# DIVE128/DMVSNet

Measured on AMD Instinct MI355X. Metric: depth-maps/sec, DTU 1600x1184 5-view 3-stage (64/32/8 hyp), higher is better.
Workload: dtype f32; 1 GPU; BASELINE configs[1]: 1600x1184, 5 views, 64/32/8 hypotheses, 3 stage(s) x (main + 4-plane refine); parallelism=1 GPU, k1=warp_corr_q4 (quad-planar features, one launch configuration per shape), conv_backend=auto, streams=2, maps_in_flight=1, hip_graph=False

## Files before the change

### dmvsnet_amd/csrc/common.h

```cpp
#pragma once
#include <hip/hip_runtime.h>
#include <stdint.h>
#include "../../include/dmvs.h"

#define DMVS_LAUNCH_CHECK()                         \
    do {                                            \
        hipError_t e__ = hipGetLastError();         \
        return e__ == hipSuccess ? 0 : (int)e__;    \
    } while (0)

static inline int ceil_div(int a, int b) { return (a + b - 1) / b; }

int dmvs_ensure_dynamic_lds(const void* kernel, size_t lds_bytes);

typedef float float4_t __attribute__((ext_vector_type(4)));
typedef float float2_t __attribute__((ext_vector_type(2)));

static inline unsigned xcd_grid(int ntiles) { return 8u * (unsigned)((ntiles + 7) / 8); }

static inline double wino_filter(const double g[9], int i, int p) {
    static const double Gm[4][3] = {{1, 0, 0}, {0.5, 0.5, 0.5}, {0.5, -0.5, 0.5}, {0, 0, 1}};
    double u = 0.0;
    for (int ky = 0; ky < 3; ++ky)
        for (int kx = 0; kx < 3; ++kx) u += Gm[i][ky] * Gm[p][kx] * g[ky * 3 + kx];
    return u;
}

enum { DMVS_ZFORM_S1 = 0, DMVS_ZFORM_S2 = 1, DMVS_ZFORM_T2 = 2 };
#ifdef __HIPCC__
__host__ __device__
#endif
constexpr unsigned zpad_live_mask(int form, int D, int oz0, int TZ) {
    unsigned m = 0;
    for (int p = 0; p < TZ; ++p) {
        const int z = oz0 + p;
        const int nplanes = form == DMVS_ZFORM_S2 ? (D + 1) / 2 : D;
        if (z < 0 || z >= nplanes) continue;
        for (int kz = 0; kz < 3; ++kz) {
            const int iz = form == DMVS_ZFORM_S1 ? z + kz - 1 : form == DMVS_ZFORM_S2 ? 2 * z + kz - 1 : (kz == 0 ? z + 1 : z);
            if (iz >= 0 && iz < D) m |= 1u << (3 * p + kz);
        }
    }
    return m;
}

constexpr int kZpadMaxDepth = 4;
extern long g_zpad_skip;
static inline bool zpad_skip_wanted(int D) { return g_zpad_skip && D <= kZpadMaxDepth; }

#ifdef __HIPCC__
__device__ __forceinline__ bool xcd_tile(int nx, int ny, int nz, bool z_fast, int& bx, int& by, int& bz) {
    const int n = nx * ny * nz, per = (n + 7) >> 3;
    const int id = blockIdx.x, t = (id & 7) * per + (id >> 3);
    if (t >= n) return false;
    bx = t % nx;
    const int r = t / nx;
    if (z_fast) { bz = r % nz; by = r / nz; } else { by = r % ny; bz = r / ny; }
    return true;
}
#endif
```

### dmvsnet_amd/csrc/conv3d_mfma.hip

```cpp
#ifndef DMVS_KO
#define DMVS_KO 0
#endif
#ifndef DMVS_X
#define DMVS_X 0
#endif
#include "common.h"
#include "tile_loader.h"

#include <algorithm>
#include <cstdlib>
#include <mutex>


#include <map>
#include <type_traits>
#include <utility>

int dmvs_ensure_dynamic_lds(const void* kernel, size_t lds_bytes) {
    static std::mutex mu;
    static std::map<std::pair<int, const void*>, size_t> configured;
    int dev = 0;
    if (hipGetDevice(&dev) != hipSuccess) return (int)hipGetLastError();
    std::lock_guard<std::mutex> lock(mu);
    auto key = std::make_pair(dev, kernel);
// ... 61 lines not shown
    }
    static __device__ __forceinline__ int row(int r, int lk) { return lk * 4 + r; }
};

template <int NROWS>
__device__ __forceinline__ void load_weights(__amdgpu_buffer_rsrc_t rs_w, float* wl, int chunk, int wave, int lane) {
    constexpr int NI = (NROWS + 3) / 4;
    const unsigned base = (unsigned)chunk * NROWS * 256u + (unsigned)lane * 16u;
#pragma unroll
    for (int r = 0; r < (NI + 3) / 4; ++r) {
        const int j = min(wave + 4 * r, NI - 1);
        if (j * 256 + lane * 4 < NROWS * 64)
            __builtin_amdgcn_raw_ptr_buffer_load_lds(rs_w, (lds_ptr_t)(wl + j * 256), 16, base + (unsigned)j * 1024u, 0, 0, 0);
    }
}

template <int M, int STRIDE, int KD, int KS, int CI_CH, int TZ, int TY, bool V4>
struct ConvGeom {
    static constexpr int KK = Frag<M>::KK;
    static constexpr int NT = KS * KS * KD;
    static constexpr int IZ = KD == 3 ? (TZ - 1) * STRIDE + 3 : TZ, IY = (TY - 1) * STRIDE + KS, IX = 31 * STRIDE + KS;
    static constexpr int XOFF = V4 && KS > 1 ? 4 - KS / 2 : 0;
    static constexpr int IXP = V4 ? (XOFF + IX + 3) / 4 * 4 : IX + 1;
    static constexpr int LPR = IXP / 4;
    static constexpr int PS0 = IZ * IY * IXP;
    static constexpr int BANK = M == 16 ? 16 : 32;
    static constexpr int PS = V4 ? PS0 + (BANK - PS0 % 64 + 64) % 64 : PS0;
    static constexpr int GPC = CI_CH / KK;
    static constexpr int TPG = CI_CH < KK ? KK / CI_CH : 1;
    static constexpr int NSTEPS = CI_CH < KK ? (NT + TPG - 1) / TPG : NT * GPC;
    static constexpr int TILE_F = (CI_CH * PS + 63) & ~63;
};

template <int M, int MB, int STRIDE, int KD, int KS, int CI_CH, int TZ, int TY, int ROWS, bool V4, bool MBS = false, unsigned ZDEAD = 0>
__global__ __launch_bounds__(256, (M == 16 ? 3 : 1)) void conv_mfma_kernel(ConvArgs a) {
    static_assert(!ZDEAD || (KD == 3 && KS == 3), "only the 3x3x3 layers have depth taps");
    typedef Frag<M> F;
    typedef typename F::acc_t acc_t;
    typedef ConvGeom<M, STRIDE, KD, KS, CI_CH, TZ, TY, V4> G;
    constexpr int PAD = KS / 2;
    constexpr int XB = 32 / F::NV;
    constexpr int SZ = KD == 3 ? STRIDE : 1;
    constexpr int IZ = G::IZ, IY = G::IY, IX = G::IX, IXP = G::IXP, PS = G::PS, GPC = G::GPC;
    constexpr int WROWS = G::NSTEPS * MB;
    constexpr int BUF_F = G::TILE_F + WROWS * 64;
    constexpr bool PACKED = CI_CH < F::KK;
    constexpr bool TR = M == 16;
    static_assert(TZ * TY == (MBS ? 2 : 4) * ROWS, "tile rows must equal the row-owning waves x ROWS");
    static_assert(!MBS || MB == 2, "M-block split: two-block layers only");
    constexpr int MBL = MBS ? 1 : MB;
    static_assert(PACKED ? (F::KK % CI_CH == 0) : (CI_CH % F::KK == 0), "channel chunk vs MFMA k-group");
    extern __shared__ __attribute__((aligned(16))) float smem[];

    const int tid = threadIdx.x, lane = tid & 63;
    const int wave = __builtin_amdgcn_readfirstlane(tid >> 6);
    const int ln = lane % F::NV, lk = lane / F::NV;
    const int rwave = MBS ? (wave >> 1) : wave;
    const int mb0 = MBS ? (wave & 1) : 0;
    int bx, by, bz;
    if (!xcd_tile(a.nx, a.ny, a.nz, KD == 3, bx, by, bz)) return;
    const int ox0 = bx * 32, oy0 = by * TY, oz0 = bz * TZ;
    const int ix0 = ox0 * STRIDE - PAD, iy0 = oy0 * STRIDE - PAD, iz0 = KD == 3 ? oz0 * STRIDE - 1 : oz0;
    if (DMVS_X & 8) {
        switch ((blockIdx.x >> 3) & 3) {
            case 1: __builtin_amdgcn_s_setprio(1); break;
            case 2: __builtin_amdgcn_s_setprio(2); break;
            case 3: __builtin_amdgcn_s_setprio(3); break;
            default: break;
        }
// ... 17 lines not shown
        for (int st = 0; st < G::NSTEPS; ++st) {
            int toff = 0;
#pragma unroll
            for (int q = 0; q < TPG; ++q) {
                const int t = st * TPG + q < NT ? st * TPG + q : NT - 1;
                const int o = ((t / (KS * KS)) * IY + (t / KS) % KS) * IXP + t % KS;
                toff = (tsel == q) ? o : toff;
            }
            ptap[st] = boff[0][0] + toff;
            asm volatile("" : "+v"(ptap[st]));
        }
    }

    acc_t acc[MBL][ROWS][XB];
#pragma unroll
    for (int mb = 0; mb < MBL; ++mb)
#pragma unroll
        for (int i = 0; i < ROWS; ++i)
#pragma unroll
            for (int xb = 0; xb < XB; ++xb)
#pragma unroll
                for (int r = 0; r < F::ACC; ++r) acc[mb][i][xb][r] = 0.f;

    const int in_vol = a.D * a.H * a.W;
    auto chunk_rsrc = [&](int ci0, int nch) {
        if (a.in_cs)
            return __builtin_amdgcn_make_buffer_rsrc((void*)(a.in + (size_t)ci0 * a.in_cs), (short)0, (a.in_elems - ci0 * a.in_cs) * 4, 0x00020000);
        return __builtin_amdgcn_make_buffer_rsrc((void*)(a.in + (size_t)ci0 * in_vol), (short)0, nch * in_vol * 4, 0x00020000);
    };
    const int nchunks = a.Cin / CI_CH;
    const __amdgpu_buffer_rsrc_t rs_w =
        __builtin_amdgcn_make_buffer_rsrc((void*)a.w, (short)0, nchunks * WROWS * 256, 0x00020000);

    auto stage = [&](int c, float* dst) {
        if (!(DMVS_KO & 1)) {
            if constexpr (V4)
                load_tile4<CI_CH, IZ, IY, G::LPR, PS>(a.D, a.H, a.W, chunk_rsrc(c * CI_CH, CI_CH), dst, iz0, iy0, ix0 - G::XOFF, wave, lane, a.in_cs, a.in_zs);
            else
                load_tile<CI_CH, IZ, IY, IX, IXP, PS, true>(a.D, a.H, a.W, chunk_rsrc(c * CI_CH, CI_CH), dst, c * CI_CH, iz0, iy0, ix0, wave, lane, a.in_cs, a.in_zs);
        }
        load_weights<WROWS>(rs_w, dst + G::TILE_F, c, wave, lane);
    };
    float sc_tr[TR ? MBL : 1], sh_tr[TR ? MBL : 1];
    if constexpr (TR && !(DMVS_X & 1)) {
#pragma unroll
        for (int mb = 0; mb < MBL; ++mb) {
            const int co = (mb0 + mb) * M + ln;
            const bool cok = co < a.Cout;
            sc_tr[mb] = (a.scale && cok) ? a.scale[co] : 1.f;
            sh_tr[mb] = (a.scale && cok) ? a.shift[co] : 0.f;
        }
    }
    K3_TR(0, K3_NOW());
    K3_TR_HW();
    [[maybe_unused]] unsigned long long tr_wait = 0, tr_mfma = 0, tr_t = K3_NOW();
    stage(0, smem);
    for (int c = 0; c < nchunks; ++c) {
        asm volatile("s_waitcnt vmcnt(0)" ::: "memory");
        __syncthreads();
#ifdef DMVS_K3_TRACE
        { const unsigned long long n = K3_NOW(); tr_wait += n - tr_t; tr_t = n; if (c == 0) K3_TR(1, n); }
#endif
        float* cur = smem + (a.single_buf ? 0 : (c & 1)) * BUF_F;
        if (c + 1 < nchunks && !a.single_buf) {
            stage(c + 1, smem + ((c + 1) & 1) * BUF_F);
        }
        const float* tile = cur;
        const float* wl = cur + G::TILE_F + lane;
        if constexpr (PACKED) {
// ... 451 lines not shown
    {16, 16, DMVS_CONV_S1, 1, 16, 1, CI_F1},
    {16, 32, DMVS_CONV2D_K5S2, 1, 32, 1, CI_K5B},
    {32, 32, DMVS_CONV_S1, 1, 32, 1, CI_F2},
    {32, 16, DMVS_CONV_S1, 1, 16, 1, CI_FO3},
    {32, 64, DMVS_CONV2D_K1, 1, 32, 2, CI_K1},
    {16, 32, DMVS_CONV2D_K1, 1, 32, 1, CI_K1},
    {8, 32, DMVS_CONV2D_K1, 1, 32, 1, CI_K1},
};

int taps_of(int mode, int kdepth) {
    return mode == DMVS_CONV2D_K5S2 ? 25 : mode == DMVS_CONV2D_K1 ? 1 : 9 * kdepth;
}

const Cfg* find_cfg(int cin, int cout, int mode, int kdepth) {
    for (const Cfg& c : kCfgs)
        if (c.cin == cin && c.cout == cout && c.mode == mode && c.kd == kdepth) return &c;
    return nullptr;
}

int tap_of(int p, int o) { return p == 0 ? 1 : (o == 0 ? 2 : 0); }

#define kMinBlocks g_min_blocks

template <typename K>
int launch_with_lds(K kernel, dim3 tiles, size_t lds_bytes, ConvArgs a, hipStream_t st) {
    a.nx = tiles.x; a.ny = tiles.y; a.nz = tiles.z;
    a.st4 = a.Wo % 4 == 0 && (reinterpret_cast<uintptr_t>(a.out) & 15) == 0;
    const dim3 grid(xcd_grid(tiles.x * tiles.y * tiles.z));
    if (int e = dmvs_ensure_dynamic_lds(reinterpret_cast<const void*>(kernel), lds_bytes)) return e;
    kernel<<<grid, 256, lds_bytes, st>>>(a);
    DMVS_LAUNCH_CHECK();
}

template <int M, int MB, int STRIDE, int KD, int KS, int CI_CH, int TZ, int TY, bool V4, bool MBS = false, unsigned ZDEAD = 0>
int launch_conv_tile_v(const ConvArgs& a, hipStream_t st) {
    if constexpr (KD == 3 && KS == 3 && STRIDE == 2 && TZ == 1 && V4 && ZDEAD == 0)
        if (zpad_skip_wanted(a.D) && a.Do == 1 && (~zpad_live_mask(DMVS_ZFORM_S2, a.D, 0, 1) & 7u) == 1u)
            return launch_conv_tile_v<M, MB, STRIDE, KD, KS, CI_CH, TZ, TY, V4, MBS, 1u>(a, st);
    typedef ConvGeom<M, STRIDE, KD, KS, CI_CH, TZ, TY, V4> G;
    constexpr int ROWS = TZ * TY / (MBS ? 2 : 4);
    constexpr size_t lds2 = 2 * (size_t)(G::TILE_F + G::NSTEPS * MB * 64) * sizeof(float);
    static_assert(lds2 <= 160 * 1024, "two pipeline stages must fit the 160 KB LDS");
    ConvArgs b = a;
    dim3 grid(ceil_div(a.Wo, 32), ceil_div(a.Ho, TY), ceil_div(a.Do, TZ));
    b.single_buf = (KD == 3 && (long)grid.x * grid.y * grid.z >= g_single_buf_min_blocks) ? 1 : 0;
    return launch_with_lds(conv_mfma_kernel<M, MB, STRIDE, KD, KS, CI_CH, TZ, TY, ROWS, V4, MBS, ZDEAD>, grid, b.single_buf ? lds2 / 2 : lds2, b, st);
}

inline bool can_v4(const ConvArgs& a) { return a.W % 4 == 0 && (reinterpret_cast<uintptr_t>(a.in) & 15) == 0; }

template <int M, int MB, int STRIDE, int KD, int KS, int CI_CH, int TZ, int TY, bool MBS = false>
int launch_conv_tile(const ConvArgs& a, hipStream_t st) {
    return can_v4(a) ? launch_conv_tile_v<M, MB, STRIDE, KD, KS, CI_CH, TZ, TY, true, MBS>(a, st)
                     : launch_conv_tile_v<M, MB, STRIDE, KD, KS, CI_CH, TZ, TY, false, MBS>(a, st);
}

#define kSplitBlocks g_split_blocks
constexpr int kPlanMBS = 1 << 17;
inline int conv_tile_choice(int stride, int kd, int Do, int Ho, int Wo, int MB) {
    const bool flat = (kd == 1) || Do == 1;
    const int big_ty_flat = (stride == 1) ? 16 : 8, big_ty = (stride == 1) ? 8 : 4;
    const long big_blocks = flat ? (long)ceil_div(Wo, 32) * ceil_div(Ho, big_ty_flat) * Do
                                 : (long)ceil_div(Wo, 32) * ceil_div(Ho, big_ty) * ceil_div(Do, 2);
    const bool big = big_blocks >= kMinBlocks;
    if (!big && MB == 2) {
        const long small_blocks = flat ? (long)ceil_div(Wo, 32) * ceil_div(Ho, 4) * Do
                                       : (long)ceil_div(Wo, 32) * ceil_div(Ho, 2) * ceil_div(Do, 2);
        if (small_blocks < kSplitBlocks) return kPlanMBS | (flat ? 256 + 2 : 2 * 256 + 1);
    }
    if (flat) return 256 + (big ? big_ty_flat : 4);
    return 2 * 256 + (big ? big_ty : 2);
}

template <int M, int MB, int STRIDE, int KD, int CI_CH, int KS = 3>
int launch_conv(const ConvArgs& a, hipStream_t st) {
    constexpr int BIG_TY_FLAT = (STRIDE == 1) ? 16 : 8, BIG_TY = (STRIDE == 1) ? 8 : 4;
    const int choice = conv_tile_choice(STRIDE, KD, a.Do, a.Ho, a.Wo, MB);
    const int tz = (choice >> 8) & 255, ty = choice & 255;
    if constexpr (MB == 2) {
// ... 184 lines not shown
```

### dmvsnet_amd/csrc/conv3d_wino.hip

```cpp
#ifndef DMVS_WKO
#define DMVS_WKO 0
#endif
#include "common.h"
#include "tile_loader.h"
#include "wino.h"
#include "dev_guard.h"

#include <algorithm>
#include <cmath>
#include <vector>

extern long g_wino_stages, g_wino_persistent, g_wino_conv0_grid;
namespace {

constexpr bool kNoStores = (DMVS_WKO & 4) != 0;
#if DMVS_WKO & 2
__device__ __forceinline__ acc4_t wino_mfma(float a, float b, acc4_t c) { c.x += a + b; return c; }
#else
__device__ __forceinline__ acc4_t wino_mfma(float a, float b, acc4_t c) { return __builtin_amdgcn_mfma_f32_16x16x4f32(a, b, c, 0, 0, 0); }
#endif

struct WinoArgs {
    const float* in;
    float* out;
// ... 227 lines not shown
#pragma unroll
                for (int oz = 0; oz < TZ; ++oz)
#pragma unroll
                    for (int t = 0; t < TRW; ++t) {
                        float row[2][8];
#pragma unroll
                        for (int r = 0; r < 4; ++r) wino_out_xform(acc[oz][t][mb], r, row[0] + 2 * r, row[1] + 2 * r);
                        const int oz_g = oz0 + oz;
#pragma unroll
                        for (int rr = 0; rr < 2; ++rr) {
                            const int oy = oy0 + 2 * (TRW * trg + t) + rr;
                            const bool rok = cok && oz_g < a.D && oy < a.H;
#pragma unroll
                            for (int h = 0; h < 2; ++h) {
                                const int x = ox0 + 8 * lk + 4 * h;
                                const unsigned pos = (unsigned)(co * out_vol + oz_g * out_plane + oy * a.W + x) * 4u;
                                v4u_t qv;
                                qv.x = wino_bn_relu(row[rr][4 * h + 0], sc[mb][0], sh[mb][0], lo);
                                qv.y = wino_bn_relu(row[rr][4 * h + 1], sc[mb][0], sh[mb][0], lo);
                                qv.z = wino_bn_relu(row[rr][4 * h + 2], sc[mb][0], sh[mb][0], lo);
                                qv.w = wino_bn_relu(row[rr][4 * h + 3], sc[mb][0], sh[mb][0], lo);
                                wino_store16<kNoStores>(rs_out, qv, (rok && x < a.W) ? pos : kInvalid);
                            }
                        }
                    }
            }
        }
        if (!has_next) break;
        cur = nxt;
        vb += (int)gridDim.x;
    }
}

__global__ __launch_bounds__(256, 2) void conv0_wino_kernel(WinoArgs a) {
    constexpr int TZ = 2, TY = 8, IZ = 4, IY = 10, LPR = 10, IXP = 40;
    constexpr int PS0 = IZ * IY * IXP, PS = PS0 + (32 - PS0 % 64 + 64) % 64;
    constexpr int TILE_F = (2 * PS + 63) & ~63, W_F = 2 * 4 * 256;
    constexpr unsigned kInvalid = kWinoInvalid;
    extern __shared__ __attribute__((aligned(16))) float smem[];

    const int tid = threadIdx.x, lane = tid & 63;
    const int wave = __builtin_amdgcn_readfirstlane(tid >> 6);
    const int ln = lane & 15, lk = lane >> 4;
    struct Tile { int ox0, oy0, oz0; };
    const XcdTileWalk walk(a.nx * a.ny * a.nz);
    auto tile_of = [&](int vb, Tile& t) {
        int id;
        if (!walk.id_of(vb, id)) return false;
        const int bx = id % a.nx, r = id / a.nx;
        t.ox0 = bx * 32; t.oz0 = (r % a.nz) * TZ; t.oy0 = (r / a.nz) * TY;
        return true;
    };
    int vb = blockIdx.x;
    Tile cur, nxt;
    if (!tile_of(vb, cur)) return;

    const int in_vol = a.D * a.H * a.W;
    const __amdgpu_buffer_rsrc_t rs_in = __builtin_amdgcn_make_buffer_rsrc((void*)a.in, (short)0, 2 * in_vol * 4, 0x00020000);
    const __amdgpu_buffer_rsrc_t rs_w = __builtin_amdgcn_make_buffer_rsrc((void*)a.w, (short)0, W_F * 4, 0x00020000);
    float* const tiles = smem + W_F;
    auto stage = [&](const Tile& t, float* dst) {
        if (DMVS_WKO & 1) return;
        load_tile4<2, IZ, IY, LPR, PS>(a.D, a.H, a.W, rs_in, dst, t.oz0 - 1, t.oy0 - 1, t.ox0 - 4, wave, lane);
    };
    const int pbase = (lk & 1) * PS + (2 * wave) * IXP + 2 + 2 * ln;
    const int zsel = lk >> 1;
    const float* wl = smem + lane * 4;

    const int co = ln;
    const float sc = a.scale ? a.scale[co] : 1.f, sh = a.scale ? a.shift[co] : 0.f;
    const int out_plane = a.H * a.W, out_vol = a.D * out_plane;
    const __amdgpu_buffer_rsrc_t rs_out = __builtin_amdgcn_make_buffer_rsrc((void*)a.out, (short)0, a.Cout * out_vol * 4, 0x00020000);
    const float lo = a.relu ? 0.f : -INFINITY;

    load_rows64<W_F / 64>(rs_w, smem, 0, wave, lane);
    stage(cur, tiles);
    for (int k = 0;; ++k) {
        const bool has_next = tile_of(vb + (int)gridDim.x, nxt);
        asm volatile("s_waitcnt vmcnt(0)" ::: "memory");
        __syncthreads();
        if (has_next) stage(nxt, tiles + ((k + 1) & 1) * TILE_F);
        const float* tile = tiles + (k & 1) * TILE_F + pbase;
        acc4_t acc[TZ][16];
#pragma unroll
        for (int oz = 0; oz < TZ; ++oz)
#pragma unroll
            for (int st = 0; st < 2; ++st) {
                const float* p = tile + (oz + (st ? 2 : zsel)) * (IY * IXP);
                float d[4][4];
                wino_read_patch(p, IXP, d);
                float v[16];
#pragma unroll
                for (int x = 0; x < 4; ++x) wino_bt4(d[0][x], d[1][x], d[2][x], d[3][x], d[0][x], d[1][x], d[2][x], d[3][x]);
#pragma unroll
                for (int y = 0; y < 4; ++y) wino_bt4(d[y][0], d[y][1], d[y][2], d[y][3], v[4 * y], v[4 * y + 1], v[4 * y + 2], v[4 * y + 3]);
#pragma unroll
// ... 6 lines not shown
                        acc[oz][4 * q + e] = wino_mfma(v[4 * q + e], wv4[e], c0);
                    }
                }
            }
#pragma unroll
        for (int oz = 0; oz < TZ; ++oz) {
            float row[2][8];
#pragma unroll
            for (int r = 0; r < 4; ++r) wino_out_xform(acc[oz], r, row[0] + 2 * r, row[1] + 2 * r);
            const int oz_g = cur.oz0 + oz;
#pragma unroll
            for (int rr = 0; rr < 2; ++rr) {
                const int oy = cur.oy0 + 2 * wave + rr;
                const bool rok = oz_g < a.D && oy < a.H;
#pragma unroll
                for (int h = 0; h < 2; ++h) {
                    const int x = cur.ox0 + 8 * lk + 4 * h;
                    const unsigned pos = (unsigned)(co * out_vol + oz_g * out_plane + oy * a.W + x) * 4u;
                    v4u_t qv;
                    qv.x = wino_bn_relu(row[rr][4 * h + 0], sc, sh, lo);
                    qv.y = wino_bn_relu(row[rr][4 * h + 1], sc, sh, lo);
                    qv.z = wino_bn_relu(row[rr][4 * h + 2], sc, sh, lo);
                    qv.w = wino_bn_relu(row[rr][4 * h + 3], sc, sh, lo);
                    wino_store16<kNoStores>(rs_out, qv, (rok && x < a.W) ? pos : kInvalid);
                }
            }
        }
        if (!has_next) break;
        cur = nxt;
        vb += (int)gridDim.x;
    }
}

template <bool Q4>
__global__ __launch_bounds__(512, 2) void fpn_wino_kernel(WinoArgs a, const float* ones) {
    constexpr int IY = 18, IXP = 40, LPR = 10, PS = 736, PPP = PS / 4;
    constexpr int TD_IXP = 24, TD_LPR = 6, TD_PS = 240, TD_PPP = 60;
    constexpr int LAT_F = 9 * PS, TD_F = 32 * TD_PS, STAGE_F = LAT_F + TD_F;
    constexpr int WL_F = 3 * 4 * 256, WT_F = 8 * 3 * 256, W_F = WL_F + WT_F;
    constexpr int NI_LAT = (9 * PPP + 63) / 64, NI_TD = (32 * TD_PPP + 63) / 64, NI = NI_LAT + NI_TD;
    static_assert((8 * PPP) % 64 == 0, "the ones plane starts on an instruction boundary");
    constexpr unsigned kInvalid = kWinoInvalid;
    extern __shared__ __attribute__((aligned(16))) float smem[];

    const int tid = threadIdx.x, lane = tid & 63;
    const int wave = __builtin_amdgcn_readfirstlane(tid >> 6);
    const int ln = lane & 15, lk = lane >> 4;
    struct Tile { int ox0, oy0, z; };
    const XcdTileWalk walk(a.nx * a.ny * a.nz);
    auto tile_of = [&](int vb, Tile& t) {
        int id;
        if (!walk.id_of(vb, id)) return false;
        const int bx = id % a.nx, r = id / a.nx;
        t.ox0 = bx * 32; t.oy0 = (r % a.ny) * 16; t.z = r / a.ny;
        return true;
    };
    int vb = blockIdx.x;
    Tile cur, nxt;
    if (!tile_of(vb, cur)) return;

    const int plane = a.H * a.W, in_vol = a.D * plane;
    const int tdH = a.H >> 1, tdW = a.W >> 1, td_plane = tdH * tdW, td_vol = a.D * td_plane;
    const __amdgpu_buffer_rsrc_t rs_lat = __builtin_amdgcn_make_buffer_rsrc((void*)a.lat, (short)0, 8 * in_vol * 4, 0x00020000);
    const __amdgpu_buffer_rsrc_t rs_one = __builtin_amdgcn_make_buffer_rsrc((void*)ones, (short)0, plane * 4, 0x00020000);
    const __amdgpu_buffer_rsrc_t rs_td = __builtin_amdgcn_make_buffer_rsrc((void*)a.td, (short)0, 32 * td_vol * 4, 0x00020000);
    const __amdgpu_buffer_rsrc_t rs_w = __builtin_amdgcn_make_buffer_rsrc((void*)a.w, (short)0, W_F * 4, 0x00020000);
    float* const stages = smem + W_F;
    constexpr int NJ = (NI + 7) / 8;
    int s_rel[NJ], s_rc[NJ];
#pragma unroll
    for (int j = 0; j < NJ; ++j) {
        const int i = wave + 8 * j;
        if (i < NI_LAT) {
            const int p = i * 64 + lane, pl = p / PPP, r = p - pl * PPP, row = r / LPR, pc = r - row * LPR;
            const bool one = i >= 8 * PPP / 64;
            s_rel[j] = (one ? 0 : pl * in_vol) + row * a.W + 4 * pc;
            s_rc[j] = row | (4 * pc) << 8 | ((pl < 9 && row < IY) ? 1 << 16 : 0) | (p < 9 * PPP ? 1 << 17 : 0);
        } else {
            const int it = i - NI_LAT;
            const int p = it * 64 + lane, pl = p / TD_PPP, r = p - pl * TD_PPP, row = r / TD_LPR, pc = r - row * TD_LPR;
            s_rel[j] = pl * td_vol + row * tdW + 4 * pc;
            s_rc[j] = row | (4 * pc) << 8 | ((i < NI && pl < 32) ? 3 << 16 : 0);
        }
    }
    auto stage = [&](const Tile& t, float* dst) {
        if (DMVS_WKO & 1) return;
        const int lat0 = t.z * plane + (t.oy0 - 1) * a.W + t.ox0 - 4, td0 = t.z * td_plane + ((t.oy0 >> 1) - 1) * tdW + (t.ox0 >> 1) - 4;
#pragma unroll
        for (int j = 0; j < NJ; ++j) {
            const int i = wave + 8 * j;
            if (i >= NI) break;
            const int row = s_rc[j] & 255, col = (s_rc[j] >> 8) & 255;
            if (i < NI_LAT) {
                const int gy = t.oy0 - 1 + row, gx = t.ox0 - 4 + col;
                const bool ok = (s_rc[j] & (1 << 16)) && (unsigned)gy < (unsigned)a.H && (unsigned)gx < (unsigned)a.W;
                const bool one = i >= 8 * PPP / 64;
                const unsigned off = ok ? (unsigned)(s_rel[j] + (one ? lat0 - t.z * plane : lat0)) * 4u : kInvalid;
                if (s_rc[j] & (1 << 17)) {
                    if (one) __builtin_amdgcn_raw_ptr_buffer_load_lds(rs_one, (lds_ptr_t)(dst + i * 256), 16, off, 0, 0, 0);
                    else __builtin_amdgcn_raw_ptr_buffer_load_lds(rs_lat, (lds_ptr_t)(dst + i * 256), 16, off, 0, 0, 0);
                }
            } else {
                const int gy = (t.oy0 >> 1) - 1 + row, gx = (t.ox0 >> 1) - 4 + col;
                const bool ok = (s_rc[j] & (1 << 16)) && (unsigned)gy < (unsigned)tdH && (unsigned)gx < (unsigned)tdW;
                __builtin_amdgcn_raw_ptr_buffer_load_lds(rs_td, (lds_ptr_t)(dst + LAT_F + (i - NI_LAT) * 256), 16,
                                                         ok ? (unsigned)(s_rel[j] + td0) * 4u : kInvalid, 0, 0, 0);
            }
        }
    };
    for (int j = wave; j < W_F / 256; j += 8)
        __builtin_amdgcn_raw_ptr_buffer_load_lds(rs_w, (lds_ptr_t)(smem + j * 256), 16, (unsigned)(j * 1024 + lane * 16), 0, 0, 0);

    constexpr int NCO = Q4 ? 4 : 1;
    float sc[NCO], sh[NCO];
#pragma unroll
    for (int r = 0; r < NCO; ++r) {
        const int co = Q4 ? 4 * lk + r : ln;
        sc[r] = a.scale ? a.scale[co] : 1.f;
        sh[r] = a.scale ? a.shift[co] : 0.f;
    }
// ... 124 lines not shown
        vb += (int)gridDim.x;
    }
}

}
long g_wino_stages = 0;
long g_wino_persistent = 1;
long g_wino_conv0_grid = 512;
namespace {

template <int KD, int MB, int MBW, int TZ, int TRW, int GPC, bool Q4 = false, bool ZSKIP = false>
int launch_wino(WinoArgs a, bool single_buf, hipStream_t st) {
    if constexpr (KD == 3 && TZ == 2 && !ZSKIP)
        if (zpad_skip_wanted(a.D)) return launch_wino<KD, MB, MBW, TZ, TRW, GPC, Q4, true>(a, single_buf, st);
    typedef WinoGeom<KD, MB, MBW, TZ, TRW, GPC> G;
    constexpr size_t lds2 = 2 * (size_t)G::BUF_F * sizeof(float);
    static_assert(lds2 / 2 <= 160 * 1024, "one stage must fit the LDS");
    a.nx = ceil_div(a.W, 32); a.ny = ceil_div(a.H, G::TY); a.nz = ceil_div(a.D, TZ);
    if (g_wino_stages) single_buf = g_wino_stages == 1;
    a.single_buf = (single_buf || lds2 > 160 * 1024) ? 1 : 0;
    const size_t lds = a.single_buf ? lds2 / 2 : lds2;
    auto kernel = conv_wino_kernel<KD, MB, MBW, TZ, TRW, GPC, Q4, ZSKIP>;
    if (int e = dmvs_ensure_dynamic_lds(reinterpret_cast<const void*>(kernel), lds)) return e;
    const unsigned resident = 256u * (unsigned)std::max<size_t>(1, std::min<size_t>(2, (160 * 1024) / lds));
    const unsigned grid = std::min(xcd_grid(a.nx * a.ny * a.nz), g_wino_persistent ? resident : 0xffffffffu);
    kernel<<<dim3(grid), 256, lds, st>>>(a);
    DMVS_LAUNCH_CHECK();
}

int launch_conv0_wino(WinoArgs a, bool, hipStream_t st) {
    constexpr int PS0 = 4 * 10 * 40, PS = PS0 + (32 - PS0 % 64 + 64) % 64;
    constexpr size_t lds = (2 * 4 * 256 + 2 * (size_t)((2 * PS + 63) & ~63)) * sizeof(float);
    a.nx = ceil_div(a.W, 32); a.ny = ceil_div(a.H, 8); a.nz = ceil_div(a.D, 2);
    if (int e = dmvs_ensure_dynamic_lds(reinterpret_cast<const void*>(conv0_wino_kernel), lds)) return e;
    const unsigned grid = std::min(xcd_grid(a.nx * a.ny * a.nz), g_wino_persistent ? (unsigned)g_wino_conv0_grid : 0xffffffffu);
    conv0_wino_kernel<<<dim3(grid), 256, lds, st>>>(a);
    DMVS_LAUNCH_CHECK();
}

typedef int (*WinoLaunch)(WinoArgs, bool single_buf, hipStream_t);
struct WCfg {
    int cin, cout, kd;
    bool flat;
    int MB, GPC;
    int TZ, TY;
    bool single_buf;
    WinoLaunch launch[2];
    long ksteps() const { return GPC ? (long)cin / 4 * kd : 2; }
};
template <int KD, int MB, int MBW, int TZ, int TRW, int GPC>
constexpr WCfg wino_row(int cin, int cout, bool flat, bool single_buf) {
    return {cin, cout, KD, flat, MB, GPC, TZ, WinoGeom<KD, MB, MBW, TZ, TRW, GPC>::TY, single_buf,
            {launch_wino<KD, MB, MBW, TZ, TRW, GPC, false>, launch_wino<KD, MB, MBW, TZ, TRW, GPC, true>}};
}
const WCfg kWCfgs[] = {
    wino_row<3, 1, 1, 1, 2, 1>(16, 16, true, true),
    wino_row<3, 1, 1, 2, 1, 1>(16, 16, false, true),
    wino_row<3, 2, 2, 1, 1, 1>(32, 32, false, true),
    wino_row<3, 4, 2, 1, 1, 1>(64, 64, false, true),
    wino_row<1, 4, 2, 1, 1, 1>(64, 64, false, true),
    wino_row<1, 1, 1, 1, 2, 2>(16, 16, false, false),
    wino_row<1, 2, 2, 1, 1, 2>(32, 32, false, false),
    {2, 16, 3, false, 1, 0, 2, 8, false, {launch_conv0_wino, nullptr}},
    wino_row<1, 1, 1, 1, 2, 1>(32, 16, false, false),
};

const WCfg* find_wcfg(int cin, int cout, int kd, int D = 0) {
    for (const WCfg& c : kWCfgs)
        if (c.cin == cin && c.cout == cout && c.kd == kd && (!c.flat || D == 1)) return &c;
// ... 91 lines not shown
    for (int gk = 0; gk < 8; ++gk)
        for (int q = 0; q < 3; ++q)
            for (int l = 0; l < 64; ++l)
                for (int e = 0; e < 4; ++e) {
                    const int j = 4 * q + e, co = l % 16, ci = 4 * gk + l / 16;
                    if (j >= 9) { out[n++] = 0.f; continue; }
                    const int ya = pos[j / 3], xb = pos[j % 3];
                    double g[9];
                    for (int t = 0; t < 9; ++t) g[t] = w3[((size_t)co * Cin + ci) * 9 + t];
                    out[n++] = (float)(wino_filter(g, ya, xb) * (ya == 1 ? 2.0 : 1.0) * (xb == 1 ? 2.0 : 1.0));
                }
    (void)Cout;
    return n == (size_t)dmvs_conv3d_wino_fpn_weight_floats() ? 0 : DMVS_EINVAL;
}

extern "C" int dmvs_conv3d_wino_fpn2(const float* lat, const float* td, const float* ones_hw, float* out, const float* w_packed,
                                     const float* scale, const float* shift, int D, int H, int W, int flags,
                                     dmvs_stream_t stream) {
    if (!lat || !td || !ones_hw || !out || !w_packed || D < 1 || H < 2 || W < 8) return DMVS_EINVAL;
    if ((scale == nullptr) != (shift == nullptr)) return DMVS_EINVAL;
    if (flags & ~(DMVS_RELU | DMVS_OUT_Q4)) return DMVS_EUNSUPPORTED;
    if ((H & 1) || (W & 7)) return DMVS_EUNSUPPORTED;
    if (((reinterpret_cast<uintptr_t>(lat) | reinterpret_cast<uintptr_t>(td) | reinterpret_cast<uintptr_t>(out) |
          reinterpret_cast<uintptr_t>(ones_hw)) & 15) != 0) return DMVS_EUNSUPPORTED;
    if ((long)16 * D * H * W >= (1L << 29)) return DMVS_EUNSUPPORTED;
    WinoArgs a = {};
    a.lat = lat; a.td = td; a.out = out; a.w = w_packed; a.scale = scale; a.shift = shift;
    a.Cin = 32; a.Cout = 16; a.D = D; a.H = H; a.W = W; a.relu = (flags & DMVS_RELU) ? 1 : 0;
    a.nx = ceil_div(W, 32); a.ny = ceil_div(H, 16); a.nz = D;
    constexpr size_t lds = ((3 * 4 + 8 * 3) * 256 + 2 * (size_t)(9 * 736 + 32 * 240)) * sizeof(float);
    static_assert(lds <= 160 * 1024, "filters + two stages must fit the LDS");
    hipStream_t st = (hipStream_t)stream;
    const unsigned grid = std::min(xcd_grid(a.nx * a.ny * a.nz), 256u);
    if (flags & DMVS_OUT_Q4) {
        if (int e = dmvs_ensure_dynamic_lds(reinterpret_cast<const void*>(fpn_wino_kernel<true>), lds)) return e;
        fpn_wino_kernel<true><<<dim3(grid), 512, lds, st>>>(a, ones_hw);
    } else {
        if (int e = dmvs_ensure_dynamic_lds(reinterpret_cast<const void*>(fpn_wino_kernel<false>), lds)) return e;
        fpn_wino_kernel<false><<<dim3(grid), 512, lds, st>>>(a, ones_hw);
    }
    DMVS_LAUNCH_CHECK();
}
```

### dmvsnet_amd/csrc/layout.hip

```cpp
#include "common.h"

#include <cstring>

template <int C>
__global__ __launch_bounds__(256) void nchw_to_hwc_kernel(const float* __restrict__ src, long chan_stride, int c0, int HW,
                                                          float* __restrict__ dst) {
    __shared__ float tile[C * 257];
    const int p0 = blockIdx.x * 256;
    const int t = threadIdx.x;
    const int np = min(256, HW - p0);
    if (t < np) {
#pragma unroll
        for (int c = 0; c < C; ++c) tile[c * 257 + t] = src[(size_t)(c0 + c) * chan_stride + p0 + t];
    }
    __syncthreads();
    const int total = np * C;
    float* out = dst + (size_t)p0 * C;
#pragma unroll
    for (int k = 0; k < C; ++k) {
        const int i = k * 256 + t;
        if (i < total) out[i] = tile[(i % C) * 257 + (i / C)];
    }
}

// ... 271 lines not shown

extern "C" int dmvs_hypotheses_next(const float* last, int h, int w, const float* dv, int n, float ratio, int D,
                                    int inverse, float* out, float* out_itv, dmvs_stream_t s) {
    return hyp_next_launch(last, h, w, 2, dv, n, ratio, D, inverse, out, out_itv, D, s);
}

extern "C" int dmvs_hypotheses_next_up(const float* last, int h, int w, int up, const float* dv, int n, float ratio, int D,
                                       int inverse, int base_only, float* out, float* out_itv, dmvs_stream_t s) {
    if (base_only && inverse) return DMVS_EINVAL;
    return hyp_next_launch(last, h, w, up, dv, n, ratio, D, inverse, out, out_itv, base_only ? 1 : D, s);
}

extern "C" int dmvs_hypothesis_base_first(const float* dv, int n, int D, int H, int W, float* base_hw, float* out_itv,
                                          dmvs_stream_t s) {
    if (!dv || !base_hw || !out_itv || n < 2 || D < 2 || H <= 0 || W <= 0) return DMVS_EINVAL;
    dim3 grid(ceil_div(W, 256), H, 1);
    hyp_first_kernel<<<grid, 256, 0, (hipStream_t)s>>>(dv, n, D, H, W, 0, base_hw, out_itv);
    DMVS_LAUNCH_CHECK();
}

extern "C" int dmvs_hypothesis_base_next(const float* last, int h, int w, const float* dv, int n, float ratio, int D,
                                         float* base_hw, float* out_itv, dmvs_stream_t s) {
    return hyp_next_launch(last, h, w, 2, dv, n, ratio, D, 0, base_hw, out_itv, 1, s);
}

extern "C" int dmvs_version(void) { return DMVS_VERSION; }

extern long g_single_buf_min_blocks;
extern long g_min_blocks, g_split_blocks, g_wino_stages, g_wino_persistent, g_wino_conv0_grid, g_deconv_prefetch;
extern long g_c8_rows;
extern long g_k3r_grid, g_k3r_counted_wait;
extern long g_k3z_grid, g_k3z_zs;
long g_zpad_skip = 1;

extern "C" long dmvs_zpad_live_mask(int form, int D, int oz0, int TZ) {
    if (form < DMVS_ZFORM_S1 || form > DMVS_ZFORM_T2 || D < 1 || oz0 < 0 || TZ < 1 || TZ > 10) return -1;
    return (long)zpad_live_mask(form, D, oz0, TZ);
}

extern "C" int dmvs_tune(const char* name, int value) {
    if (!name) return DMVS_EINVAL;
    if (!strcmp(name, "k3_single_buf_min_blocks")) { if (value < 0) return DMVS_EINVAL; g_single_buf_min_blocks = value; return 0; }
    if (!strcmp(name, "k3_min_blocks")) { if (value < 0) return DMVS_EINVAL; g_min_blocks = value; return 0; }
    if (!strcmp(name, "k3_split_blocks")) { if (value < 0) return DMVS_EINVAL; g_split_blocks = value; return 0; }
    if (!strcmp(name, "wino_conv0_grid")) { if (value < 8 || value % 8) return DMVS_EINVAL; g_wino_conv0_grid = value; return 0; }
    if (!strcmp(name, "k3_deconv_prefetch")) { g_deconv_prefetch = value ? 1 : 0; return 0; }
    if (!strcmp(name, "c8_rows")) { if (value < 0 || value > 4096) return DMVS_EINVAL; g_c8_rows = value; return 0; }
    if (!strcmp(name, "wino_persistent")) { g_wino_persistent = value ? 1 : 0; return 0; }
    if (!strcmp(name, "k3r_grid")) { if (value < 32 || value > 1024 || value % 32) return DMVS_EINVAL; g_k3r_grid = value; return 0; }
    if (!strcmp(name, "k3z_grid")) { if (value < 0 || value > 4096 || value % 8) return DMVS_EINVAL; g_k3z_grid = value; return 0; }
    if (!strcmp(name, "k3z_zs")) { if (value < 0 || value > 64) return DMVS_EINVAL; g_k3z_zs = value; return 0; }
    if (!strcmp(name, "k3r_counted_wait")) { g_k3r_counted_wait = value ? 1 : 0; return 0; }
    if (!strcmp(name, "zpad_skip")) { if (value != 0 && value != 1) return DMVS_EINVAL; g_zpad_skip = value; return 0; }
    if (!strcmp(name, "wino_stages")) { if (value < 0 || value > 2) return DMVS_EINVAL; g_wino_stages = value; return 0; }
    return DMVS_EUNSUPPORTED;
}

extern "C" const char* dmvs_error_string(int code) {
    if (code == 0) return "ok";
    if (code == DMVS_EINVAL) return "dmvs: invalid argument";
    if (code == DMVS_EUNSUPPORTED) return "dmvs: unsupported channel count or mode";
    if (code > 0) return hipGetErrorString((hipError_t)code);
    return "dmvs: unknown error";
}
```

### dmvsnet_amd/csrc/tile_loader.h

```cpp
#pragma once
#include "common.h"

typedef __attribute__((address_space(3))) void* lds_ptr_t;
#ifndef DMVS_TILE_AUX
#define DMVS_TILE_AUX 0
#endif

template <int CI_CH, int IZ, int IY, int IX, int IXP, int PS, bool NEG>
__device__ __forceinline__ void load_tile(int aD, int aH, int aW, __amdgpu_buffer_rsrc_t rsrc, float* tile, int ci0,
                                          int iz0, int iy0, int ix0, int wave, int lane, int cs = 0, int zs = 0) {
    constexpr int MW = IX < 64 ? IX : 64;
    constexpr int YI = (IY + 3) / 4;
    constexpr unsigned kInvalid = 0x80000000u, kInvalidX = 0x40000000u;
    const int plane = zs ? zs : aH * aW, vol = cs ? cs : aD * aH * aW;
    const int gx = ix0 + lane;
    const bool xin = (!NEG || gx >= 0) && gx < aW;
    const unsigned gx4 = xin ? (unsigned)gx * 4u : kInvalidX;
    int yoff[YI], ly[YI];
    bool yin[YI];
#pragma unroll
    for (int k = 0; k < YI; ++k) {
        const int y = min(wave + 4 * k, IY - 1), gy = iy0 + y;
        yin[k] = (!NEG || gy >= 0) && gy < aH;
        yoff[k] = gy * aW;
        ly[k] = y * IXP;
    }
    if (lane < MW) {
#pragma unroll
        for (int c = 0; c < CI_CH; ++c) {
#pragma unroll
            for (int z = 0; z < IZ; ++z) {
                const int gz = iz0 + z;
                const bool zin = (!NEG || gz >= 0) && gz < aD;
                const int cz = c * vol + gz * plane;
// ... 25 lines not shown
    }
}


template <int CI_CH, int IZ, int IY, int LPR, int PS>
__device__ __forceinline__ void load_tile4(int aD, int aH, int aW, __amdgpu_buffer_rsrc_t rsrc, float* tile, int iz0,
                                           int iy0, int ix0a, int wave, int lane, int cs = 0, int zs = 0) {
    constexpr int RPI = 64 / LPR;
    constexpr int NR = IZ * IY;
    constexpr int G = (NR + RPI - 1) / RPI;
    constexpr int IXP = 4 * LPR;
    constexpr unsigned kInvalid = 0x80000000u;
    const int plane = zs ? zs : aH * aW, vol = cs ? cs : aD * aH * aW;
    const int lr = lane / LPR, x4 = lane - lr * LPR;
    const int gx = ix0a + 4 * x4;
    const bool xin = (unsigned)gx < (unsigned)aW;
#pragma unroll
    for (int k = 0; k < (G + 3) / 4; ++k) {
        const int g = min(wave + 4 * k, G - 1);
        const int r = g * RPI + lr;
        const int z = r / IY, y = r - z * IY;
        const int gz = iz0 + z, gy = iy0 + y;
        const bool ok = xin && (unsigned)gz < (unsigned)aD && (unsigned)gy < (unsigned)aH;
        const int rel = gz * plane + gy * aW + gx;
        if (lr < RPI && r < NR) {
#pragma unroll
            for (int c = 0; c < CI_CH; ++c) {
                const unsigned off = ok ? (unsigned)(c * vol + rel) * 4u : kInvalid;
                __builtin_amdgcn_raw_ptr_buffer_load_lds(rsrc, (lds_ptr_t)(tile + c * PS + g * RPI * IXP), 16, off, 0, 0, DMVS_TILE_AUX);
            }
        }
    }
}
```

Measured before the change: 94.56 depth-maps/s.

## Add precomputed-lane 16-byte tile loader with packed byte-range bounds checks

Introduces a Tile4Lanes loader that computes each lane's relative offsets and packed tile coordinates once per kernel. Per stage it does a single packed range check against the tile box and passes the per-channel offset as a scalar soffset, instead of recomputing divisions and bounds and per-channel vector offsets on every stage. The loader is wired into the stride-2 3x3x3 MFMA conv, the conv0 Winograd kernel and the FPN Winograd kernel, and is on by default behind a runtime flag. The gain is lower address-generation ALU and VGPR cost in the load path. The cost is more kernel template instantiations and extra registers held across the loop.

```diff
diff --git a/dmvsnet_amd/csrc/common.h b/dmvsnet_amd/csrc/common.h
--- a/dmvsnet_amd/csrc/common.h
+++ b/dmvsnet_amd/csrc/common.h
@@ -46,6 +46,7 @@
 
 constexpr int kZpadMaxDepth = 4;
 extern long g_zpad_skip;
+extern long g_tile_loader_v2;
 static inline bool zpad_skip_wanted(int D) { return g_zpad_skip && D <= kZpadMaxDepth; }
 
 #ifdef __HIPCC__
diff --git a/dmvsnet_amd/csrc/conv3d_mfma.hip b/dmvsnet_amd/csrc/conv3d_mfma.hip
--- a/dmvsnet_amd/csrc/conv3d_mfma.hip
+++ b/dmvsnet_amd/csrc/conv3d_mfma.hip
@@ -117,9 +117,10 @@
     static constexpr int TILE_F = (CI_CH * PS + 63) & ~63;
 };
 
-template <int M, int MB, int STRIDE, int KD, int KS, int CI_CH, int TZ, int TY, int ROWS, bool V4, bool MBS = false, unsigned ZDEAD = 0>
+template <int M, int MB, int STRIDE, int KD, int KS, int CI_CH, int TZ, int TY, int ROWS, bool V4, bool MBS = false, unsigned ZDEAD = 0, bool LV2 = false>
 __global__ __launch_bounds__(256, (M == 16 ? 3 : 1)) void conv_mfma_kernel(ConvArgs a) {
     static_assert(!ZDEAD || (KD == 3 && KS == 3), "only the 3x3x3 layers have depth taps");
+    static_assert(!LV2 || V4, "the 16-byte loader");
     typedef Frag<M> F;
     typedef typename F::acc_t acc_t;
     typedef ConvGeom<M, STRIDE, KD, KS, CI_CH, TZ, TY, V4> G;
@@ -203,9 +204,15 @@
     const __amdgpu_buffer_rsrc_t rs_w =
         __builtin_amdgcn_make_buffer_rsrc((void*)a.w, (short)0, nchunks * WROWS * 256, 0x00020000);
 
+    typedef Tile4Lanes<CI_CH, LV2 ? IZ : 0, IY, G::LPR, PS> TL;
+    [[maybe_unused]] const TL tl(a.in_zs ? a.in_zs : a.H * a.W, a.W, (a.in_cs ? a.in_cs : in_vol) * 4, wave, lane);
+    [[maybe_unused]] unsigned tvoff[TL::NK + 1];
+    if constexpr (LV2) tl.place(a.D, a.H, a.W, a.in_zs ? a.in_zs : a.H * a.W, iz0, iy0, ix0 - G::XOFF, tvoff);
     auto stage = [&](int c, float* dst) {
         if (!(DMVS_KO & 1)) {
-            if constexpr (V4)
+            if constexpr (LV2)
+                tl.issue(chunk_rsrc(c * CI_CH, CI_CH), dst, tvoff, wave);
+            else if constexpr (V4)
                 load_tile4<CI_CH, IZ, IY, G::LPR, PS>(a.D, a.H, a.W, chunk_rsrc(c * CI_CH, CI_CH), dst, iz0, iy0, ix0 - G::XOFF, wave, lane, a.in_cs, a.in_zs);
             else
                 load_tile<CI_CH, IZ, IY, IX, IXP, PS, true>(a.D, a.H, a.W, chunk_rsrc(c * CI_CH, CI_CH), dst, c * CI_CH, iz0, iy0, ix0, wave, lane, a.in_cs, a.in_zs);
@@ -723,11 +730,13 @@
     DMVS_LAUNCH_CHECK();
 }
 
-template <int M, int MB, int STRIDE, int KD, int KS, int CI_CH, int TZ, int TY, bool V4, bool MBS = false, unsigned ZDEAD = 0>
+template <int M, int MB, int STRIDE, int KD, int KS, int CI_CH, int TZ, int TY, bool V4, bool MBS = false, unsigned ZDEAD = 0, bool LV2 = false>
 int launch_conv_tile_v(const ConvArgs& a, hipStream_t st) {
+    if constexpr (KD == 3 && KS == 3 && STRIDE == 2 && M == 32 && MB == 1 && V4 && !LV2)
+        if (g_tile_loader_v2) return launch_conv_tile_v<M, MB, STRIDE, KD, KS, CI_CH, TZ, TY, V4, MBS, ZDEAD, true>(a, st);
     if constexpr (KD == 3 && KS == 3 && STRIDE == 2 && TZ == 1 && V4 && ZDEAD == 0)
         if (zpad_skip_wanted(a.D) && a.Do == 1 && (~zpad_live_mask(DMVS_ZFORM_S2, a.D, 0, 1) & 7u) == 1u)
-            return launch_conv_tile_v<M, MB, STRIDE, KD, KS, CI_CH, TZ, TY, V4, MBS, 1u>(a, st);
+            return launch_conv_tile_v<M, MB, STRIDE, KD, KS, CI_CH, TZ, TY, V4, MBS, 1u, LV2>(a, st);
     typedef ConvGeom<M, STRIDE, KD, KS, CI_CH, TZ, TY, V4> G;
     constexpr int ROWS = TZ * TY / (MBS ? 2 : 4);
     constexpr size_t lds2 = 2 * (size_t)(G::TILE_F + G::NSTEPS * MB * 64) * sizeof(float);
@@ -735,7 +744,7 @@
     ConvArgs b = a;
     dim3 grid(ceil_div(a.Wo, 32), ceil_div(a.Ho, TY), ceil_div(a.Do, TZ));
     b.single_buf = (KD == 3 && (long)grid.x * grid.y * grid.z >= g_single_buf_min_blocks) ? 1 : 0;
-    return launch_with_lds(conv_mfma_kernel<M, MB, STRIDE, KD, KS, CI_CH, TZ, TY, ROWS, V4, MBS, ZDEAD>, grid, b.single_buf ? lds2 / 2 : lds2, b, st);
+    return launch_with_lds(conv_mfma_kernel<M, MB, STRIDE, KD, KS, CI_CH, TZ, TY, ROWS, V4, MBS, ZDEAD, LV2>, grid, b.single_buf ? lds2 / 2 : lds2, b, st);
 }
 
 inline bool can_v4(const ConvArgs& a) { return a.W % 4 == 0 && (reinterpret_cast<uintptr_t>(a.in) & 15) == 0; }
diff --git a/dmvsnet_amd/csrc/conv3d_wino.hip b/dmvsnet_amd/csrc/conv3d_wino.hip
--- a/dmvsnet_amd/csrc/conv3d_wino.hip
+++ b/dmvsnet_amd/csrc/conv3d_wino.hip
@@ -283,6 +283,7 @@
     }
 }
 
+template <bool LV2>
 __global__ __launch_bounds__(256, 2) void conv0_wino_kernel(WinoArgs a) {
     constexpr int TZ = 2, TY = 8, IZ = 4, IY = 10, LPR = 10, IXP = 40;
     constexpr int PS0 = IZ * IY * IXP, PS = PS0 + (32 - PS0 % 64 + 64) % 64;
@@ -310,9 +311,17 @@
     const __amdgpu_buffer_rsrc_t rs_in = __builtin_amdgcn_make_buffer_rsrc((void*)a.in, (short)0, 2 * in_vol * 4, 0x00020000);
     const __amdgpu_buffer_rsrc_t rs_w = __builtin_amdgcn_make_buffer_rsrc((void*)a.w, (short)0, W_F * 4, 0x00020000);
     float* const tiles = smem + W_F;
+    typedef Tile4Lanes<2, LV2 ? IZ : 0, IY, LPR, PS> TL;
+    [[maybe_unused]] const TL tl(a.H * a.W, a.W, in_vol * 4, wave, lane);
     auto stage = [&](const Tile& t, float* dst) {
         if (DMVS_WKO & 1) return;
-        load_tile4<2, IZ, IY, LPR, PS>(a.D, a.H, a.W, rs_in, dst, t.oz0 - 1, t.oy0 - 1, t.ox0 - 4, wave, lane);
+        if constexpr (LV2) {
+            unsigned voff[TL::NK + 1];
+            tl.place(a.D, a.H, a.W, a.H * a.W, t.oz0 - 1, t.oy0 - 1, t.ox0 - 4, voff);
+            tl.issue(rs_in, dst, voff, wave);
+        } else {
+            load_tile4<2, IZ, IY, LPR, PS>(a.D, a.H, a.W, rs_in, dst, t.oz0 - 1, t.oy0 - 1, t.ox0 - 4, wave, lane);
+        }
     };
     const int pbase = (lk & 1) * PS + (2 * wave) * IXP + 2 + 2 * ln;
     const int zsel = lk >> 1;
@@ -385,7 +394,7 @@
     }
 }
 
-template <bool Q4>
+template <bool Q4, bool LV2>
 __global__ __launch_bounds__(512, 2) void fpn_wino_kernel(WinoArgs a, const float* ones) {
     constexpr int IY = 18, IXP = 40, LPR = 10, PS = 736, PPP = PS / 4;
     constexpr int TD_IXP = 24, TD_LPR = 6, TD_PS = 240, TD_PPP = 60;
@@ -420,7 +429,9 @@
     const __amdgpu_buffer_rsrc_t rs_w = __builtin_amdgcn_make_buffer_rsrc((void*)a.w, (short)0, W_F * 4, 0x00020000);
     float* const stages = smem + W_F;
     constexpr int NJ = (NI + 7) / 8;
+    typedef ByteRange<2> YX;
     int s_rel[NJ], s_rc[NJ];
+    [[maybe_unused]] bool s_on[NJ];
 #pragma unroll
     for (int j = 0; j < NJ; ++j) {
         const int i = wave + 8 * j;
@@ -429,16 +440,52 @@
             const bool one = i >= 8 * PPP / 64;
             s_rel[j] = (one ? 0 : pl * in_vol) + row * a.W + 4 * pc;
             s_rc[j] = row | (4 * pc) << 8 | ((pl < 9 && row < IY) ? 1 << 16 : 0) | (p < 9 * PPP ? 1 << 17 : 0);
+            if constexpr (LV2) {
+                s_rc[j] = (pl < 9 && row < IY) ? YX::pack(row, 4 * pc) : YX::kNever;
+                s_on[j] = p < 9 * PPP;
+            }
         } else {
             const int it = i - NI_LAT;
             const int p = it * 64 + lane, pl = p / TD_PPP, r = p - pl * TD_PPP, row = r / TD_LPR, pc = r - row * TD_LPR;
             s_rel[j] = pl * td_vol + row * tdW + 4 * pc;
             s_rc[j] = row | (4 * pc) << 8 | ((i < NI && pl < 32) ? 3 << 16 : 0);
-        }
+            if constexpr (LV2) {
+                s_rc[j] = (i < NI && pl < 32) ? YX::pack(row, 4 * pc) : YX::kNever;
+                s_on[j] = true;
+            }
+        }
+        if constexpr (LV2) s_rel[j] *= 4;
     }
     auto stage = [&](const Tile& t, float* dst) {
         if (DMVS_WKO & 1) return;
         const int lat0 = t.z * plane + (t.oy0 - 1) * a.W + t.ox0 - 4, td0 = t.z * td_plane + ((t.oy0 >> 1) - 1) * tdW + (t.ox0 >> 1) - 4;
+        if constexpr (LV2) {
+            unsigned yl, yh, xl, xh;
+            tile_box(t.oy0 - 1, IY, a.H, yl, yh);
+            tile_box(t.ox0 - 4, IXP, a.W, xl, xh);
+            const unsigned lat_lo = YX::pack(yl, xl), lat_hg = YX::pack_hi(yh, xh);
+            tile_box((t.oy0 >> 1) - 1, 10, tdH, yl, yh);
+            tile_box((t.ox0 >> 1) - 4, TD_IXP, tdW, xl, xh);
+            const unsigned td_lo = YX::pack(yl, xl), td_hg = YX::pack_hi(yh, xh);
+            const unsigned lat0b = (unsigned)lat0 * 4u, one0b = (unsigned)(lat0 - t.z * plane) * 4u, td0b = (unsigned)td0 * 4u;
+#pragma unroll
+            for (int j = 0; j < NJ; ++j) {
+                const int i = wave + 8 * j;
+                if (i >= NI) break;
+                if (i < NI_LAT) {
+                    const bool one = i >= 8 * PPP / 64;
+                    const unsigned off = YX::in_range((unsigned)s_rc[j], lat_lo, lat_hg) ? (unsigned)s_rel[j] + (one ? one0b : lat0b) : kInvalid;
+                    if (s_on[j]) {
+                        if (one) __builtin_amdgcn_raw_ptr_buffer_load_lds(rs_one, (lds_ptr_t)(dst + i * 256), 16, off, 0, 0, 0);
+                        else __builtin_amdgcn_raw_ptr_buffer_load_lds(rs_lat, (lds_ptr_t)(dst + i * 256), 16, off, 0, 0, 0);
+                    }
+                } else {
+                    const unsigned off = YX::in_range((unsigned)s_rc[j], td_lo, td_hg) ? (unsigned)s_rel[j] + td0b : kInvalid;
+                    __builtin_amdgcn_raw_ptr_buffer_load_lds(rs_td, (lds_ptr_t)(dst + LAT_F + (i - NI_LAT) * 256), 16, off, 0, 0, 0);
+                }
+            }
+            return;
+        }
 #pragma unroll
         for (int j = 0; j < NJ; ++j) {
             const int i = wave + 8 * j;
@@ -629,9 +676,10 @@
     constexpr int PS0 = 4 * 10 * 40, PS = PS0 + (32 - PS0 % 64 + 64) % 64;
     constexpr size_t lds = (2 * 4 * 256 + 2 * (size_t)((2 * PS + 63) & ~63)) * sizeof(float);
     a.nx = ceil_div(a.W, 32); a.ny = ceil_div(a.H, 8); a.nz = ceil_div(a.D, 2);
-    if (int e = dmvs_ensure_dynamic_lds(reinterpret_cast<const void*>(conv0_wino_kernel), lds)) return e;
+    auto kernel = g_tile_loader_v2 ? conv0_wino_kernel<true> : conv0_wino_kernel<false>;
+    if (int e = dmvs_ensure_dynamic_lds(reinterpret_cast<const void*>(kernel), lds)) return e;
     const unsigned grid = std::min(xcd_grid(a.nx * a.ny * a.nz), g_wino_persistent ? (unsigned)g_wino_conv0_grid : 0xffffffffu);
-    conv0_wino_kernel<<<dim3(grid), 256, lds, st>>>(a);
+    kernel<<<dim3(grid), 256, lds, st>>>(a);
     DMVS_LAUNCH_CHECK();
 }
 
@@ -789,12 +837,9 @@
     static_assert(lds <= 160 * 1024, "filters + two stages must fit the LDS");
     hipStream_t st = (hipStream_t)stream;
     const unsigned grid = std::min(xcd_grid(a.nx * a.ny * a.nz), 256u);
-    if (flags & DMVS_OUT_Q4) {
-        if (int e = dmvs_ensure_dynamic_lds(reinterpret_cast<const void*>(fpn_wino_kernel<true>), lds)) return e;
-        fpn_wino_kernel<true><<<dim3(grid), 512, lds, st>>>(a, ones_hw);
-    } else {
-        if (int e = dmvs_ensure_dynamic_lds(reinterpret_cast<const void*>(fpn_wino_kernel<false>), lds)) return e;
-        fpn_wino_kernel<false><<<dim3(grid), 512, lds, st>>>(a, ones_hw);
-    }
+    auto kernel = (flags & DMVS_OUT_Q4) ? (g_tile_loader_v2 ? fpn_wino_kernel<true, true> : fpn_wino_kernel<true, false>)
+                                        : (g_tile_loader_v2 ? fpn_wino_kernel<false, true> : fpn_wino_kernel<false, false>);
+    if (int e = dmvs_ensure_dynamic_lds(reinterpret_cast<const void*>(kernel), lds)) return e;
+    kernel<<<dim3(grid), 512, lds, st>>>(a, ones_hw);
     DMVS_LAUNCH_CHECK();
 }
diff --git a/dmvsnet_amd/csrc/layout.hip b/dmvsnet_amd/csrc/layout.hip
--- a/dmvsnet_amd/csrc/layout.hip
+++ b/dmvsnet_amd/csrc/layout.hip
@@ -327,6 +327,7 @@
 extern long g_k3r_grid, g_k3r_counted_wait;
 extern long g_k3z_grid, g_k3z_zs;
 long g_zpad_skip = 1;
+long g_tile_loader_v2 = 1;
 
 extern "C" long dmvs_zpad_live_mask(int form, int D, int oz0, int TZ) {
     if (form < DMVS_ZFORM_S1 || form > DMVS_ZFORM_T2 || D < 1 || oz0 < 0 || TZ < 1 || TZ > 10) return -1;
@@ -347,6 +348,7 @@
     if (!strcmp(name, "k3z_zs")) { if (value < 0 || value > 64) return DMVS_EINVAL; g_k3z_zs = value; return 0; }
     if (!strcmp(name, "k3r_counted_wait")) { g_k3r_counted_wait = value ? 1 : 0; return 0; }
     if (!strcmp(name, "zpad_skip")) { if (value != 0 && value != 1) return DMVS_EINVAL; g_zpad_skip = value; return 0; }
+    if (!strcmp(name, "tile_loader_v2")) { if (value != 0 && value != 1) return DMVS_EINVAL; g_tile_loader_v2 = value; return 0; }
     if (!strcmp(name, "wino_stages")) { if (value < 0 || value > 2) return DMVS_EINVAL; g_wino_stages = value; return 0; }
     return DMVS_EUNSUPPORTED;
 }
diff --git a/dmvsnet_amd/csrc/tile_loader.h b/dmvsnet_amd/csrc/tile_loader.h
--- a/dmvsnet_amd/csrc/tile_loader.h
+++ b/dmvsnet_amd/csrc/tile_loader.h
@@ -1,5 +1,6 @@
 #pragma once
 #include "common.h"
+#include "wino.h"
 
 typedef __attribute__((address_space(3))) void* lds_ptr_t;
 #ifndef DMVS_TILE_AUX
@@ -91,3 +92,67 @@
         }
     }
 }
+
+
+__device__ __forceinline__ void tile_box(int o, int ext, int size, unsigned& lo, unsigned& hi) {
+    const int l = max(0, -o), h = min(ext, size - o) - 1;
+    lo = h < l ? 0x7fu : (unsigned)l;
+    hi = h < l ? 0u : (unsigned)h;
+}
+
+template <int CI_CH, int IZ, int IY, int LPR, int PS>
+struct Tile4Lanes {
+    static constexpr int RPI = 64 / LPR, NR = IZ * IY, G = (NR + RPI - 1) / RPI, NK = (G + 3) / 4, IXP = 4 * LPR;
+    static_assert(IZ < 64 && IY < 128 && IXP <= 128, "tile coordinates are packed one per byte");
+    typedef ByteRange<3> XYZ;
+    static constexpr unsigned kInvalid = 0x80000000u;
+    unsigned rel[NK + 1], xyz[NK + 1];
+    bool on[NK + 1];
+    int so[CI_CH];
+
+    __device__ __forceinline__ Tile4Lanes(int plane, int aW, int cs4, int wave, int lane) {
+        const int lr = lane / LPR, x4 = lane - lr * LPR;
+#pragma unroll
+        for (int k = 0; k < NK; ++k) {
+            const int g = min(wave + 4 * k, G - 1);
+            const int r = g * RPI + lr;
+            const int z = r / IY, y = r - z * IY;
+            on[k] = lr < RPI && r < NR;
+            rel[k] = (unsigned)(z * plane + y * aW + 4 * x4) * 4u;
+            xyz[k] = on[k] ? XYZ::pack(4 * x4, y, z) : XYZ::kNever;
+        }
+        if constexpr (NR > 0) {
+#pragma unroll
+            for (int c = 0; c < CI_CH; ++c) {
+                so[c] = __builtin_amdgcn_readfirstlane(c * cs4);
+                asm volatile("" : "+s"(so[c]));
+            }
+        }
+    }
+    __device__ __forceinline__ void place(int aD, int aH, int aW, int plane, int iz0, int iy0, int ix0a, unsigned* voff) const {
+        unsigned xl, xh, yl, yh, zl, zh;
+        tile_box(ix0a, IXP, aW, xl, xh);
+        tile_box(iy0, IY, aH, yl, yh);
+        tile_box(iz0, IZ, aD, zl, zh);
+        const unsigned lo = XYZ::pack(xl, yl, zl), hg = XYZ::pack_hi(xh, yh, zh);
+        const unsigned origin = (unsigned)(iz0 * plane + iy0 * aW + ix0a) * 4u;
+#pragma unroll
+        for (int k = 0; k < NK; ++k) {
+            voff[k] = XYZ::in_range(xyz[k], lo, hg) ? rel[k] + origin : kInvalid;
+        }
+    }
+    __device__ __forceinline__ void issue(__amdgpu_buffer_rsrc_t rsrc, float* tile, const unsigned* voff, int wave) const {
+#pragma unroll
+        for (int k = 0; k < NK; ++k) {
+            const int g = min(wave + 4 * k, G - 1);
+            if (on[k]) {
+#pragma unroll
+                for (int c = 0; c < CI_CH; ++c) {
+                    const unsigned vo = voff[k];
+                    const int sc = so[c];
+                    __builtin_amdgcn_raw_ptr_buffer_load_lds(rsrc, (lds_ptr_t)(tile + c * PS + g * RPI * IXP), 16, vo, sc, 0, DMVS_TILE_AUX);
+                }
+            }
+        }
+    }
+};
```

Result: no change. 94.47 depth-maps/s (-0.1%).
